# jjfiv/fastrank

Measured on AMD Instinct MI355X. Metric: coordinate-ascent NDCG@10 evals/sec on MSLR-WEB30K shape, higher is better.
Workload: dtype f64; 1 GPU; synthetic MSLR-WEB30K shape: 3800000 docs x 136 features x 31000 queries, coordinate ascent NDCG@10, 32 restarts/GPU x 25 steps/coord (configs[2]); restarts_total=32, parallelism=restart-sharded x1 (dataset replicated), launcher=single process

## Files before the change

fastrank_amd/clib.py:

```python
import ctypes as C
import json
import os
from typing import Dict, List, Optional, Set

from . import _build

_MODEL_TYPES = ["SingleFeature", "Linear", "DecisionTree", "Ensemble"]


ALLREDUCE_SUM_FN = C.CFUNCTYPE(C.c_int, C.c_void_p, C.POINTER(C.c_double), C.c_size_t)


class _CResult(C.Structure):
    _fields_ = [("error_message", C.c_void_p), ("success", C.c_void_p)]


_lib = None


def _load():
    global _lib
    if _lib is not None:
        return _lib
    path = _build.LIB_PATH
# ... 52 lines not shown
        "fr_debug_lambda_gradients_opts": (vp, [vp, vp, vp, C.c_char_p, C.c_double, vp, sz, C.c_char_p, vp, vp, sz]),
        "fr_evaluate_dense": (vp, [vp, vp, vp, C.c_char_p, vp, sz, C.POINTER(vp)]),
        "fr_rank_order": (vp, [vp, vp, vp, sz, vp, sz]),
        "fr_dataset_num_queries": (sz, [vp]),
        "fr_dataset_num_instances": (sz, [vp]),
        "fr_dataset_device_info": (vp, [vp]),
        "fr_evaluate_candidates": (vp, [vp, vp, C.c_char_p, sz, vp, vp, vp, vp, vp, vp]),
        "fr_profile_enable": (None, [C.c_int]),
        "fr_profile_reset": (None, []),
        "fr_profile_json": (vp, []),
        "fr_debug_resident_bound": (C.c_double, [C.c_int, C.c_double, C.c_double, C.c_double]),
        "fr_synchronize": (C.c_int, []),
        "fr_debug_device_plan": (vp, [C.c_char_p, C.c_int, C.c_uint32, C.c_int]),
        "fr_debug_fullrank_class": (C.c_uint32, [C.c_uint32]),
        "fr_debug_restart_queue": (vp, [C.c_uint32, C.c_uint32, C.c_uint32, vp, C.c_uint32]),
        "fr_dataset_release_replicas": (sz, [vp]),
        "fr_debug_peer_copy": (vp, [C.c_int, C.c_int, sz]),
        "fr_pack_restart_records": (vp, [C.c_char_p, sz, sz, vp]),
        "fr_unpack_restart_records": (vp, [vp, sz, sz]),
        "fr_rccl_allgather": (vp, [vp, sz, vp, sz, vp]),
        "fr_debug_rccl_selftest": (vp, [C.c_int]),
        "fr_debug_walk_tiles": (vp, [vp, vp, vp, sz, vp, vp, sz, sz]),
        "fr_debug_device_form": (vp, [vp, C.c_int, C.c_char_p, vp, sz]),
    }
    for name, (restype, argtypes) in sigs.items():
        fn = getattr(L, name)
        fn.restype = restype
        fn.argtypes = argtypes
    _lib = L
    return L
# ... 283 lines not shown
```

fastrank_amd/csrc/capi.cpp:

```cpp
#include <atomic>
#include <limits>
#include <chrono>
#include <cstdio>
#include <cstdlib>
#include <cstring>
#include <fstream>

#include "../../include/fastrank.h"
#include "host.hpp"
#include "loader.hpp"
#include "lambdamart.hpp"
#include "rf_train.hpp"

using fr::FrError;
using frjson::Value;

struct CDataset {
    std::shared_ptr<fr::DatasetView> view;
};
struct CModel {
    fr::Model actual;
};
struct CQRel {
    fr::QRel actual;
// ... 137 lines not shown
    o.set("raw_evals", Value::uint(s.raw_evals));
    o.set("ticks", Value::uint(s.ticks));
    o.set("groups", Value::uint(s.groups));
    o.set("seconds", Value::number(s.seconds));
    o.set("path", Value::string(s.path));
    o.set("restarts", Value::uint(s.restarts));
    o.set("verify_pairs", Value::uint(s.verify_pairs));
    o.set("verify_redone", Value::uint(s.verify_redone));
    o.set("exact_ticks", Value::uint(s.exact_ticks));
    o.set("exact_groups", Value::uint(s.exact_groups));
    o.set("verify_redo_entries", Value::uint(s.verify_redo_entries));
    o.set("chain_runs", Value::uint(s.chain_runs));
    o.set("chain_visits", Value::uint(s.chain_visits));
    o.set("rank_slots_on", Value::uint(s.rank_slots_on));
    o.set("rank_slots_off", Value::uint(s.rank_slots_off));
    o.set("line_searches", Value::uint(s.line_searches));
    o.set("audit_values", Value::uint(s.audit_values));
    o.set("audit_mismatches", Value::uint(s.audit_mismatches));
    o.set("devices", Value::uint(s.devices));
    o.set("refills", Value::uint(s.refills));
    if (s.device >= 0) o.set("device", Value::uint((uint64_t)s.device));
    return o;
}

enum class Learner { CoordinateAscent, RandomForest, LambdaMART };

struct ParsedRequest {
    std::string measure;
    Learner learner = Learner::CoordinateAscent;
    fr::CAParams ca;
// ... 300 lines not shown
    const std::vector<double>& exchanged = rccl.ran ? via_rccl : blocks;
    std::vector<fr::RestartResult> hist = fr::unpack_restart_records(exchanged.data(), k * cap, dim, R);
    fr::TrainStats total = stats[0];
    total.rccl_set = true;
    total.rccl = rccl;
    for (size_t i = 0; i < k; i++) {
        if (i == 0) continue;
        total.useful_evals += stats[i].useful_evals, total.raw_evals += stats[i].raw_evals;
        total.ticks = std::max(total.ticks, stats[i].ticks), total.groups += stats[i].groups;
        total.restarts += stats[i].restarts, total.refills += stats[i].refills;
        total.verify_pairs += stats[i].verify_pairs, total.verify_redone += stats[i].verify_redone;
        total.line_searches += stats[i].line_searches, total.exact_ticks += stats[i].exact_ticks;
        total.exact_groups += stats[i].exact_groups, total.verify_redo_entries += stats[i].verify_redo_entries;
        total.chain_runs += stats[i].chain_runs, total.chain_visits += stats[i].chain_visits;
        total.rank_slots_on += stats[i].rank_slots_on, total.rank_slots_off += stats[i].rank_slots_off;
        total.audit_values += stats[i].audit_values, total.audit_mismatches += stats[i].audit_mismatches;
    }
    total.seconds = std::chrono::duration<double>(std::chrono::steady_clock::now() - t0).count();
    total.devices = (uint32_t)k;
    total.device = -1;
    set_last_stats(total, stats);
    return fr::ca_select(hist, rq.ca.output_ensemble);
}

fr::Model train_rf(const std::shared_ptr<fr::DatasetView>& view, const ParsedRequest& rq) {
    auto t0 = std::chrono::steady_clock::now();
    fr::Evaluator ev = fr::make_evaluator(*view, rq.measure, rq.has_qrel ? &rq.qrel : nullptr);
    fr::RFTrainer trainer(view, std::move(ev), rq.rf);
    std::vector<fr::RFTrainer::DevicePart> parts;
    if (rq.rf.num_trees > 0) {
// ... 419 lines not shown
                ticks[w]++;
                for (auto& p : live[w]) p.left--;
                live[w].erase(std::remove_if(live[w].begin(), live[w].end(), [](const Place& p) { return p.left == 0; }), live[w].end());
                fill(w);
            }
        }
        Value o = Value::object(), ord = Value::array(), tk = Value::array();
        for (uint32_t w = 0; w < n_workers; w++) {
            Value a = Value::array();
            for (uint32_t id : order[w]) a.push(Value::uint(id));
            ord.push(std::move(a));
            tk.push(Value::uint(ticks[w]));
        }
        o.set("order", std::move(ord));
        o.set("ticks", std::move(tk));
        return frjson::dump(o);
    });
}

size_t fr_dataset_release_replicas(const CDataset* dataset) {
    if (!dataset || !dataset->view) return 0;
    std::lock_guard<std::mutex> lk(api_mu_of(*dataset));
    size_t n = 0;
    for (fr::DatasetView* v = dataset->view.get(); v; v = v->parent.get()) n += v->release_replicas();
    return n;
}

const void* fr_debug_device_plan(const void* devices_csv, int device_count, uint32_t num_restarts, int primary_device) {
    return json_call([&]() {
        const std::string csv = accept_str("devices_csv", devices_csv);
// ... 684 lines not shown
```

fastrank_amd/csrc/device.hpp:

```cpp
#pragma once
#include <algorithm>
#include <cstddef>
#include <cstdint>
#include <memory>
#include <string>
#include <utility>
#include <vector>

namespace frdev {

const char* path_env(const char* name);
inline const char* pricing_env(const char* name) {
#ifdef FR_PRICING
    return path_env(name);
#else
    (void)name;
    return nullptr;
#endif
}

enum Measure : int { M_NDCG = 0, M_AP = 1, M_RR = 2 };

constexpr uint32_t WALK_TILE = 128;
struct WalkTileLayout {
// ... 45 lines not shown
            const size_t t0 = wts[u], t1 = std::min<size_t>((size_t)wts[u + 1], t0 + WT);
            const size_t lo = std::max(b, t0) - t0, hi = std::min(e, t1) - t0;
            for (size_t p = t0 + lo; p < t0 + hi; p++) {
                out.seg[p] = (uint16_t)(lo | (hi << 8));
                out.wofs[p] = (uint8_t)(p - t0);
            }
        }
    }
    return out;
}

inline double resident_err_refresh(uint32_t d, double T) { return 1.1 * (double)(d + 1) * 0x1p-53 * T; }
inline double resident_err_update(double err, double norm, double T) { return 1.002 * err / norm + 8.0 * 0x1p-53 * T * (1.0 + 1e-6); }
inline double resident_eps_extra(double err, double norm, double T) { return 1.01 * err / norm + 10.0 * 0x1p-53 * T; }

enum : int {
    FLAG_NAN_SCORE = 1,
    FLAG_ACTUAL_GT_IDEAL = 2,
};

struct HostCSR {
    size_t n = 0, d = 0, nq = 0;
    const float* x = nullptr;
    std::vector<uint32_t> perm;
    std::vector<uint32_t> qoff;
    std::vector<float> gain;
};

struct FlatTrees {
    std::vector<int32_t> fid, lhs, rhs;
// ... 62 lines not shown
    struct LsCounts {
        unsigned long long pairs = 0, redone = 0;
    };
    bool linesearch_submit(int ctx, int measure, int64_t depth, const double* norms, const std::vector<LineGroup>& groups,
                           std::string* err);
    bool linesearch_collect(int ctx, std::vector<double>* means, LsCounts* counts, std::string* err);
    bool linesearch(int measure, int64_t depth, const double* norms, const std::vector<LineGroup>& groups,
                    std::vector<double>* means, LsCounts* counts, std::string* err);
    uint64_t resident_reserve(size_t slots, std::string* err);
    bool resident_store_from_scores(uint64_t owner, size_t slot, size_t b, std::string* err);
    const std::vector<double>& column_absmax() const;
    unsigned long long exact_fallbacks() const;
    void routing_counters(unsigned long long* exact_groups, unsigned long long* redo_entries) const;
    void chain_counters(unsigned long long* runs, unsigned long long* visits, unsigned long long* ranked_on = nullptr,
                        unsigned long long* ranked_off = nullptr) const;
    void audit_counters(unsigned long long* values, unsigned long long* mismatches) const;
    bool download_last_matrix(std::vector<double>* out, size_t* ldm, std::string* err);

    struct RfActive { uint32_t tree, key, n; };
    struct RfCand { double position, importance; uint32_t ids_i, flags, pos_l, pos_r; double sum_l, sum_r; };
    struct RfSplit { int32_t fslot; uint32_t pos, left, right; };
    bool rf_set_presence(const uint32_t* bits_by_instance, size_t words, size_t n_instances, std::string* err);
    bool rf_begin(const std::vector<uint32_t>& root_off, const std::vector<uint32_t>& root_ids, uint32_t nf,
                  const std::vector<uint32_t>& feats, std::string* err, const uint32_t* positions = nullptr,
                  bool lambda_targets = false);
    bool rf_positions(const std::vector<uint32_t>& root_ids, uint32_t* positions , std::string* err);
    bool rf_root_outputs(std::vector<double>* out, std::string* err);
    bool rf_level(const std::vector<RfActive>& active, const std::vector<uint32_t>& slot_of_key, uint32_t k, int method,
                  uint32_t min_leaf, std::vector<RfCand>* cands, std::vector<float>* label_minmax, std::string* err);
    bool rf_split(const std::vector<RfSplit>& splits, std::vector<double>* child_out, std::string* err);
// ... 81 lines not shown
```

fastrank_amd/csrc/device_dataset.inc:

```

static constexpr int LS_CONTEXTS = DeviceDataset::LINESEARCH_CONTEXTS;

static double fv_class_cost(int ci) {
    static const int sort_ce[] = {63, 191, 384, 543, 849, 1056}, merge_ce[] = {32, 80, 144, 192, 304, 336};
    const uint32_t nl = FV_CLASSES[ci].nl, pl = FV_CLASSES[ci].pl;
    const int ni = (int)nl / 16 - 1;
    uint32_t rounds = 0;
    while ((1u << rounds) < pl) rounds++;
    double c = 2.0 * nl + 2.0 * sort_ce[ni] + 5.0 * nl + (double)nl * pl;
    for (uint32_t r = 1; r <= rounds; r++) c += 5.0 * r * nl + 2.0 * merge_ce[ni];
    static const double lane_penalty[] = {1.0, 1.1, 1.25, 1.6, 2.0, 2.4};
    return c * pl * lane_penalty[rounds];
}

static int fv_class_of(uint32_t len) {
    static const bool pow2_only = [] {
        const char* e = frdev::pricing_env("FR_FV_CLASSES");
        return e != nullptr && std::strcmp(e, "pow2") == 0;
    }();
    int best = -1;
    double best_cost = 0.0;
    for (int ci = 0; ci < FV_NCLASSES; ci++) {
        const uint32_t nl = FV_CLASSES[ci].nl, pl = FV_CLASSES[ci].pl, npad = nl * pl;
        if (npad < len) continue;
// ... 52 lines not shown
        LsKind kind = LSK_TOPK;
        TickStage ts;
        LSArgs a;
        RRArgs ra;
        FSArgs fsa;
        RMArgs rma;
        DevBuf<double> fv_rows;
        size_t ldm = 0, maxc = 0, lds = 0;
        int64_t depth = 0;
        int measure = 0;
        int xs_used = 1;
        bool xs_pinned = false;
        bool audit = false;
        std::vector<LineGroup> agroups;
        unsigned redo_grid = 512, redo_grid_used = 512;
        size_t nverify = 0;
        std::vector<uint32_t> gorder, gredo_h;
        std::vector<int> gslot;
        std::vector<LineGroup> pgroups;
        std::vector<double> exact_means;
        LsCounts counts;
    };
    LsCtx ls[LS_CONTEXTS + 1];
    hipEvent_t res_ready = nullptr;
    bool res_ready_set = false;
    const double* last_M = nullptr;
    DevBuf<uint32_t> sub_idx;
    DevBuf<double> sub_partial, sub_means;
    uint32_t sub_na = 0, sub_nb = 0;
    bool ls_submit(LsCtx& c, int path, int measure, int64_t depth, const double* norms, const std::vector<LineGroup>& groups,
// ... 53 lines not shown
    DevBuf<uint8_t> wofs;
    DevBuf<uint32_t> wlist;
    std::vector<uint32_t> wt_start_h;
    size_t nwt = 0, nwlist = 0;
    std::vector<double> colstd;
    std::vector<uint8_t> colmode;
    std::vector<ColStats> colstats_h;
    DevBuf<uint8_t> rslot;
    std::vector<uint16_t> slot_rank_age;
    std::vector<uint16_t> slot_rank_upd;
    std::vector<uint16_t> slot_rank_gap;
    std::vector<uint8_t> slot_rank_mode;
    std::vector<uint16_t> slot_rate_n;
    std::vector<float> slot_rate;
    unsigned long long rank_slots_on = 0, rank_slots_off = 0;
    bool build_order_tables(std::string* err);
    DevBuf<float> xcol;
    bool build_columns(std::string* err);
    DevBuf<uint16_t> gkey;
    uint32_t key_bits = 0, key_cls_bits = 0;
    uint64_t dup_groups = 0;
    DevBuf<float> xb, gain;
    DevBuf<double> gexp, disc;
    DevBuf<uint32_t> qstart, qlen, qtight, perm, rank, run_q0, run_q1, run_pos, run_docs, run_order, gcls, qlist;
    struct SizeClass {
        uint32_t npad, offset, count;
    };
    std::vector<SizeClass> size_classes;
    std::vector<SizeClass> fv_classes;
    DevBuf<uint32_t> fv_qlist;
// ... 914 lines not shown
    copy(m.run_q0, sm.run_q0, "replicate run_q0");
    copy(m.run_q1, sm.run_q1, "replicate run_q1");
    copy(m.run_pos, sm.run_pos, "replicate run_pos");
    copy(m.run_docs, sm.run_docs, "replicate run_docs");
    copy(m.run_order, sm.run_order, "replicate run_order");
    copy(m.run_lo, sm.run_lo, "replicate run_lo");
    copy(m.gcls, sm.gcls, "replicate gcls");
    copy(m.gkey, sm.gkey, "replicate gkey");
    copy(m.segtab, sm.segtab, "replicate segtab");
    copy(m.wt_start, sm.wt_start, "replicate wt_start");
    copy(m.run_wt0, sm.run_wt0, "replicate run_wt0");
    copy(m.wofs, sm.wofs, "replicate wofs");
    m.wt_start_h = sm.wt_start_h;
    m.nwt = sm.nwt;
    m.verify_xs = sm.verify_xs;
    auto copy_optional = [&](auto& dst, const auto& from, const char* what, const char* degraded) {
        if (!ok || from.p == nullptr || from.cap == 0) return;
        std::string e2;
        if (!dst.ensure(from.cap, &e2)) {
            (void)hipGetLastError();
            warn_degraded(degraded);
            return;
        }
        ok = chk(hipMemcpyPeerAsync(dst.p, device, from.p, sm.device, from.bytes(), m.stream), what);
    };
    copy_optional(m.xcol, sm.xcol, "replicate xcol", "a device replica has no HBM for the column-major copy of the matrix: its line searches form their sums from the tiles");
    copy_optional(m.xslot, sm.xslot, "replicate xslot", "a device replica has no HBM for the visiting-order tables: its NDCG@k verify kernel walks in storage order");
    m.colstd = sm.colstd;
    m.colmode = sm.colmode;
    m.colstats_h = sm.colstats_h;
// ... 136 lines not shown
    m.xslot.alias(pm.xslot);
    m.segtab.alias(pm.segtab);
    m.wt_start.alias(pm.wt_start);
    m.wofs.alias(pm.wofs);
    m.wt_start_h = pm.wt_start_h;
    m.nwt = pm.nwt;
    m.nwlist = wlist.size();
    m.xcol.alias(pm.xcol);
    m.colstd = pm.colstd;
    m.colmode = pm.colmode;
    m.colstats_h = pm.colstats_h;
    m.dup_groups = pm.dup_groups;
    m.key_bits = pm.key_bits;
    m.key_cls_bits = pm.key_cls_bits;
    m.verify_xs = pm.verify_xs;
    m.perm.alias(pm.perm);
    m.disc.alias(pm.disc);
    m.dcgtab.alias(pm.dcgtab);
    m.termtab.alias(pm.termtab);
    if (!upload(m.qstart, qstart, err) || !upload(m.qlen, qlen, err) || !upload(m.qtight, qtight, err) ||
        !upload(m.run_q0, run_q0, err) || !upload(m.run_q1, run_q1, err) || !upload(m.run_pos, run_pos, err) ||
        !upload(m.run_docs, run_docs, err) || !upload(m.run_order, run_order, err) || !upload(m.run_lo, run_lo, err) ||
        !upload(m.qlist, qlist, err) || !upload(m.fv_qlist, fv_qlist, err) || !upload(m.qnpos, qnpos, err) ||
        !upload(m.qnneg, qnneg, err) || !upload(m.vtiles, vtiles, err) || !upload(m.run_wt0, run_wt0, err) || !upload(m.wlist, wlist, err))
        return nullptr;
    m.nvtiles = frdev::pricing_env("FR_VIEW_ALL_TILES") ? 0 : vtiles.size();
    if (!m.flags.ensure(1, err) || !m.dbgc.ensure(4, err)) return nullptr;
    if (!chk(hipMemset(m.flags.p, 0, sizeof(int)), "clear flags")) return nullptr;
    m.qstart_h = qstart;
    m.qlen_h = qlen;
    m.qnpos_h = qnpos;
    m.qnneg_h = qnneg;
    return ds;
}

static bool launch_means(const double* M, size_t ldm, size_t ncols, size_t nq, bool sums_only, DevBuf<double>& partial,
                         DevBuf<double>& means, hipStream_t st, std::string* err, const void* tail_count = nullptr,
                         const int* tail_flags = nullptr, double* host_copy = nullptr, const uint32_t* tail_groups = nullptr) {
    if (tail_count != nullptr && host_copy == nullptr) return false;
    const size_t nseg = (nq + MEAN_SEG - 1) / MEAN_SEG;
    if (!partial.ensure(std::max<size_t>(1, nseg) * ldm, err) || !means.ensure(ldm + mean_tail_words(ldm), err)) return false;
    {
        ProfScope ps("segment_sum_kernel", st);
        dim3 grid((unsigned)nseg, (unsigned)((ncols + 63) / 64));
        segment_sum_kernel<<<grid, 64, 0, st>>>(M, (uint32_t)ldm, (uint32_t)ncols, (uint32_t)nq, partial.p);
    }
    {
        ProfScope ps("final_mean_kernel", st);
        final_mean_kernel<<<dim3((unsigned)((ncols + 63) / 64)), 64, 0, st>>>(partial.p, (uint32_t)ldm, (uint32_t)ncols,
                                                                              (uint32_t)nseg, (uint32_t)(sums_only ? (nq ? 1 : 0) : nq), means.p,
                                                                              static_cast<const unsigned long long*>(tail_count), tail_flags, host_copy,
                                                                              tail_groups);
    }
    FR_HIP(hipGetLastError());
    return true;
}

static inline dim3 grid1d(size_t n, unsigned bs) { return dim3((unsigned)((n + bs - 1) / bs)); }

bool DeviceDataset::score_linear(size_t B, const double* weights, std::string* err) {
    Impl& m = *impl_;
    std::lock_guard<std::mutex> lk(m.mu);
    if (!m.bind(err)) return false;
    if (B == 0) return true;
    const size_t dp = m.dq * 4;
    if (!m.scores.ensure(B * m.np, err) || !m.weights.ensure(B * dp, err)) return false;
    m.scores_slots = B;
// ... 794 lines not shown
    return true;
}

bool DeviceDataset::Impl::tick_upload(LsCtx& c, bool with_eps2, std::string* err) {
    Impl& m = *this;
    if (with_eps2) std::memcpy(c.th<double>(c.ts.o_eps2), m.eps2_host.data(), c.ts.G * 64 * sizeof(double));
    if (m.res_ready_set && c.stream != m.stream) FR_HIP(hipStreamWaitEvent(c.stream, m.res_ready, 0));
    FR_HIP(hipMemcpyAsync(c.tick_d.p, c.tick_h.p, c.ts.total, hipMemcpyHostToDevice, c.stream));
    return true;
}
bool DeviceDataset::Impl::ls_means(LsCtx& c, std::string* err) {
    Impl& m = *this;
    const size_t ldm = c.ldm;
    if (!c.tick_res.ensure((ldm + mean_tail_words(ldm)) * sizeof(double), err)) return false;
    return launch_means(c.M.p, ldm, ldm, m.nq, m.sums_only, c.partial, c.means, c.stream, err, c.td<unsigned long long>(c.ts.o_count),
                        c.flags.p, reinterpret_cast<double*>(c.tick_res.p), c.kind == LSK_TOPK ? c.td<uint32_t>(c.ts.o_gredo) : nullptr);
}

bool DeviceDataset::Impl::tick_finish(LsCtx& c, size_t ldm, std::vector<double>* means, uint32_t* nredo, std::string* err,
                                      uint32_t* npairs, std::vector<uint32_t>* by_group) {
    Impl& m = *this;
    const size_t tail = ldm * sizeof(double);
    hipStream_t st = c.stream;
    FR_HIP(hipStreamSynchronize(st));
    means->resize(ldm);
    std::memcpy(means->data(), c.tick_res.p, tail);
    unsigned long long words[2] = {0, 0};
    std::memcpy(words, c.tick_res.p + tail, sizeof(words));
    *nredo = (uint32_t)words[0];
    if (npairs) *npairs = (uint32_t)(words[0] >> 32);
    if (by_group) {
// ... 148 lines not shown
        else if (xs == 2) linesearch_verify_kernel<K, 1, true, 2><<<grid, dim3(WAVE), tab_lds, st>>>(a);
        else if (xs == 3 || K < 10) linesearch_verify_kernel<K, 1, true, 3><<<grid, dim3(WAVE), tab_lds, st>>>(a);
        else linesearch_verify_kernel<K, 1, true, (K < 10 ? 3 : 4)><<<grid, dim3(WAVE), tab_lds, st>>>(a);
    } else {
        const dim3 grid((unsigned)(nruns8 * ((G + 1) / 2)));
        linesearch_verify_kernel<K, 2, false><<<grid, dim3(WAVE), 2 * dp * sizeof(double) + tab_lds, st>>>(a);
    }
}

uint64_t DeviceDataset::resident_reserve(size_t slots, std::string* err) {
    Impl& m = *impl_;
    std::lock_guard<std::mutex> lk(m.mu);
    if (!m.bind(err)) return 0;
    m.res_owner++;
    m.verify_xs = std::max(1, m.verify_xs - 1);
    m.res_half.clear();
    if (m.xcol.p == nullptr) {
        if (err) *err = "resident_reserve: the dataset has no column-major copy";
        return 0;
    }
    m.slot_exact_left.assign(slots, 0);
    m.slot_backoff.assign(slots, 0);
    {
        std::string* e2 = err;
        auto ensure = [&]() -> bool { return m.res.ensure(slots * 2 * m.np, e2); };
        if (!ensure()) return 0;
    }
    m.res_half.assign(slots, 0);
    m.slot_rank_age.assign(slots, 0xFFFF);
    m.slot_rank_upd.assign(slots, 0);
    m.slot_rank_gap.assign(slots, 1);
    m.slot_rank_mode.assign(slots, 1);
    m.slot_rate_n.assign(slots, 0);
    m.slot_rate.assign(slots, 0.0f);
    if (m.xslot.p != nullptr) {
        std::string e2;
        if (m.rslot.ensure(slots * m.np, &e2)) {
            rslot_identity_kernel<<<dim3(1024), dim3(256), 0, m.stream>>>(m.rslot.p, m.wofs.p, m.np, slots * m.np);
            if (hipGetLastError() != hipSuccess) m.rslot.release();
        } else {
            (void)hipGetLastError();
        }
    }
    return m.res_owner;
}

bool DeviceDataset::resident_store_from_scores(uint64_t owner, size_t slot, size_t b, std::string* err) {
// ... 25 lines not shown
    *mismatches = impl_->audit_mismatches;
}

unsigned long long DeviceDataset::exact_fallbacks() const {
    std::lock_guard<std::mutex> lk(impl_->mu);
    return impl_->exact_fallbacks;
}

void DeviceDataset::chain_counters(unsigned long long* runs, unsigned long long* visits, unsigned long long* ranked_on,
                                   unsigned long long* ranked_off) const {
    std::lock_guard<std::mutex> lk(impl_->mu);
    *runs = impl_->chain_runs;
    *visits = impl_->chain_visits;
    if (ranked_on) *ranked_on = impl_->rank_slots_on;
    if (ranked_off) *ranked_off = impl_->rank_slots_off;
}

void DeviceDataset::routing_counters(unsigned long long* exact_groups, unsigned long long* redo_entries) const {
    std::lock_guard<std::mutex> lk(impl_->mu);
    *exact_groups = impl_->exact_groups;
    *redo_entries = impl_->approx_redo_entries;
}

static void launch_scores(const FSArgs& a, size_t maxc, unsigned nblocks, size_t lds, hipStream_t st) {
    if (maxc <= 16) linesearch_scores_kernel<16, 16><<<dim3(nblocks), dim3(WAVE), lds, st>>>(a);
    else if (maxc <= 51) linesearch_scores_kernel<51, 16><<<dim3(nblocks), dim3(WAVE), lds, st>>>(a);
    else linesearch_scores_kernel<64, 16><<<dim3(nblocks), dim3(WAVE), lds, st>>>(a);
}

FSArgs DeviceDataset::Impl::scores_args(const uint32_t* gf, const double* w, const double* cand, double* rows, int* fl, size_t gc) const {
// ... 743 lines not shown
    FR_HIP(hipGetLastError());
    unsigned long long bad = 0;
    FR_HIP(hipMemcpyAsync(&bad, m.audit_cnt.p, sizeof(bad), hipMemcpyDeviceToHost, m.stream));
    FR_HIP(hipStreamSynchronize(m.stream));
    m.audit_values += ncells;
    m.audit_mismatches += bad;
    return true;
}

bool DeviceDataset::Impl::topk_policy(LsCtx& c, uint32_t nredo, uint32_t nslices, std::string* err) {
    Impl& m = *this;
    const size_t ldm = c.ldm, G = ldm / 64, nV = c.nverify;
    const std::vector<uint32_t>& by_group = c.gredo_h;
    LSArgs& a = c.a;
    const unsigned grid_used = c.redo_grid_used;
    if (nredo > grid_used / 2) c.redo_grid = std::min(8192u, std::max(c.redo_grid, 512u) * 4u);
    else if (nredo < grid_used / 16 && c.redo_grid > 512u) c.redo_grid /= 2u;
    m.approx_redo_entries += nslices;
    for (size_t k = 0; k < nV; k++) m.chain_runs += by_group[G + k];
    m.chain_visits += (unsigned long long)m.n * nV;
    {
        static const double t_off = [] {
            const char* e = frdev::pricing_env("FR_RANK_OFF_BELOW");
            return e ? std::atof(e) : RANK_OFF_BELOW;
        }();
        static const double t_on = [] {
            const char* e = frdev::pricing_env("FR_RANK_ON_ABOVE");
            return e ? std::atof(e) : RANK_ON_ABOVE;
        }();
        std::vector<double> runs(m.slot_rank_mode.size(), 0.0), visits(m.slot_rank_mode.size(), 0.0);
        for (size_t k = 0; k < nV; k++) {
            const int slot = c.gslot[k];
// ... 4 lines not shown
        for (size_t slot = 0; slot < runs.size(); slot++) {
            if (visits[slot] == 0.0) continue;
            const double r = runs[slot] / visits[slot];
            uint16_t& n = m.slot_rate_n[slot];
            if (n < 16) n++;
            m.slot_rate[slot] += (float)((r - (double)m.slot_rate[slot]) / (double)n);
            if (n < 16) continue;
            if (m.slot_rank_mode[slot] == 1 && (double)m.slot_rate[slot] < t_off) {
                m.slot_rank_mode[slot] = 2;
                m.rank_slots_off++;
            } else if (m.slot_rank_mode[slot] == 2 && (double)m.slot_rate[slot] > t_on) {
                m.slot_rank_mode[slot] = 1;
                m.rank_slots_on++;
            }
        }
    }
    if (c.audit) {
        const size_t nel = m.nq * ldm;
        if (!m.audit.ensure(nel, err) || !m.audit_cnt.ensure(1, err)) return false;
        FR_HIP(hipMemcpyAsync(m.audit.p, c.M.p, nel * sizeof(double), hipMemcpyDeviceToDevice, c.stream));
        LSArgs x = a;
        x.work_list = nullptr;
        x.work_count = nullptr;
        x.g_base = 0;
        x.G = (uint32_t)G;
        dispatch_exact(x, c.depth, (unsigned)(((m.nruns + 7) / 8) * 8 * G), c.maxc, c.lds, c.stream);
        FR_HIP(hipMemsetAsync(m.audit_cnt.p, 0, sizeof(unsigned long long), c.stream));
        audit_compare_kernel<<<dim3(1024), dim3(256), 0, c.stream>>>(m.audit.p, c.M.p, nel, m.audit_cnt.p);
        unsigned long long bad = 0;
        FR_HIP(hipMemcpyAsync(&bad, m.audit_cnt.p, sizeof(bad), hipMemcpyDeviceToHost, c.stream));
// ... 1128 lines not shown
```

fastrank_amd/csrc/host.hpp:

```cpp
#pragma once
#include <algorithm>
#include <atomic>
#include <charconv>
#include <chrono>
#include <cmath>
#include <cstdint>
#include <cstdio>
#include <cstdlib>
#include <functional>
#include <map>
#include <memory>
#include <mutex>
#include <set>
#include <string>
#include <thread>
#include <unordered_map>
#include <vector>

#include "device.hpp"
#include "json.hpp"

namespace fr {

using frjson::Value;
// ... 742 lines not shown
    uint64_t useful_evals = 0;
    uint64_t raw_evals = 0;
    uint64_t ticks = 0;
    uint64_t groups = 0;
    double seconds = 0.0;
    std::string path;
    uint32_t restarts = 0;
    uint64_t verify_pairs = 0, verify_redone = 0;
    uint64_t line_searches = 0;
    uint64_t audit_values = 0, audit_mismatches = 0;
    uint64_t exact_ticks = 0;
    uint64_t exact_groups = 0;
    uint64_t verify_redo_entries = 0;
    uint64_t chain_runs = 0, chain_visits = 0;
    uint64_t rank_slots_on = 0, rank_slots_off = 0;
    uint32_t devices = 1;
    uint32_t refills = 0;
    int device = -1;
    bool rccl_set = false;
    frdev::RcclReport rccl;
};

struct ExactTickCount {
    frdev::DeviceDataset& dev;
    TrainStats& st;
    unsigned long long base, av0 = 0, am0 = 0, eg0 = 0, re0 = 0, cr0 = 0, cv0 = 0, on0 = 0, off0 = 0;
    ExactTickCount(frdev::DeviceDataset& d, TrainStats& s) : dev(d), st(s), base(d.exact_fallbacks()) {
        d.audit_counters(&av0, &am0);
        d.routing_counters(&eg0, &re0);
        d.chain_counters(&cr0, &cv0, &on0, &off0);
// ... 129 lines not shown
            path_ = caps[0] == caps[2] ? LS_TOPK : (caps[1] == caps[2] ? LS_FULLRANK : LS_NONE);
        }
        stats_.path = path_ == LS_TOPK ? "fused_linesearch" : (path_ == LS_FULLRANK ? "fused_fullrank" : "generic_sort");
        stats_.restarts = (uint32_t)rs_.size();
        if (rs_.empty()) return;
        const size_t R = rs_.size();
        std::vector<size_t> all(R);
        for (size_t k = 0; k < R; k++) all[k] = k;
        init_restarts(all);
        const char* res_env = frdev::path_env("FR_LS_RESIDENT");
        if (path_ != LS_NONE && !(res_env && res_env[0] == '0')) {
            std::string _err;
            res_owner_ = dev.resident_reserve(R, &_err);
            if (res_owner_ != 0) {
                resident_ = true;
                if (const char* e = frdev::path_env("FR_RESIDENT_REFRESH")) res_refresh_ = (uint32_t)std::max(1, atoi(e));
                for (size_t k = 0; k < R; k++) rs_[k].slot = (int)k;
                refresh_resident(all);
            }
        }
    }

    bool done() const {
        for (const Restart& r : rs_)
            if (!r.done) return false;
        return !queue_ || queue_->empty();
    }

    bool tick() {
        refill();
// ... 423 lines not shown
```

fastrank_amd/csrc/kernels_metric.inc:

```
__device__ __forceinline__ bool key_before(double sa, uint32_t ia, double sb, uint32_t ib) {
    if (ia == IDX_INVALID) return false;
    if (ib == IDX_INVALID) return true;
    if (sa > sb) return true;
    if (sa < sb) return false;
    return ia > ib;
}

__global__ __launch_bounds__(256) void metric_sort_kernel(
    const double* __restrict__ scores, uint32_t np, const uint32_t* __restrict__ qstart,
    const uint32_t* __restrict__ qlen, const uint32_t* __restrict__ qtight, const double* __restrict__ gexp,
    const float* __restrict__ gain, const double* __restrict__ disc, const double* __restrict__ norms, int measure,
    int depth, uint32_t B, double* __restrict__ M, uint32_t* __restrict__ rank_out, const uint32_t* __restrict__ perm,
    int* __restrict__ flags, uint32_t npad_max, const uint32_t* __restrict__ qlist, uint32_t b_off,
    double* gkeys, uint32_t* gidx) {
    extern __shared__ double lds_raw[];
    double* keys = lds_raw;
    uint32_t* idx = (uint32_t*)(keys + npad_max);
    if (gkeys != nullptr) {
        const size_t slab = ((size_t)blockIdx.y * gridDim.x + blockIdx.x) * npad_max;
        keys = gkeys + slab;
        idx = gidx + slab;
    }
    const uint32_t q = qlist[blockIdx.x], b = blockIdx.y + b_off, tid = threadIdx.x, nt = blockDim.x;
    const uint32_t base = qstart[q], n = qlen[q];
// ... 84 lines not shown
                        sum_precision += keys[i];
                        in_list++;
                    }
                }
                if (num_rel == 0) num_rel = in_list;
                if (num_rel != 0) result = sum_precision / (double)num_rel;
            }
        }
    }
    if (tid == 0) M[(size_t)q * B + b] = result;
}

constexpr uint32_t MEAN_SEG = 256;

__global__ __launch_bounds__(64) void segment_sum_kernel(const double* __restrict__ M, uint32_t ldm, uint32_t ncols,
                                                         uint32_t nq, double* __restrict__ partial) {
    const uint32_t c = blockIdx.y * blockDim.x + threadIdx.x;
    const uint32_t s = blockIdx.x;
    if (c >= ncols) return;
    const uint32_t q0 = s * MEAN_SEG;
    const uint32_t q1 = (q0 + MEAN_SEG < nq) ? q0 + MEAN_SEG : nq;
    const double* p = M + (size_t)q0 * ldm + c;
    double sum = 0.0;
    uint32_t q = q0;
    for (; q + 16 <= q1; q += 16) {
        double v[16];
#pragma unroll
        for (int t = 0; t < 16; t++) v[t] = p[(size_t)t * ldm];
#pragma unroll
        for (int t = 0; t < 16; t++) sum += v[t];
        p += (size_t)16 * ldm;
    }
    for (; q < q1; q++) {
        sum += *p;
        p += ldm;
    }
    partial[(size_t)s * ldm + c] = sum;
}

__host__ __device__ constexpr size_t mean_tail_words(size_t ldm) { return 2 + ldm / 64; }
__global__ void final_mean_kernel(const double* __restrict__ partial, uint32_t ldm, uint32_t ncols, uint32_t nseg,
                                  uint32_t div, double* __restrict__ means, const unsigned long long* __restrict__ tail_count,
                                  const int* __restrict__ tail_flags, double* __restrict__ host_copy,
                                  const uint32_t* __restrict__ tail_groups) {
    uint32_t c = blockIdx.x * blockDim.x + threadIdx.x;
    if (c == 0 && tail_count != nullptr) {
        const unsigned long long w0 = *tail_count, w1 = (unsigned long long)(unsigned int)*tail_flags;
        reinterpret_cast<unsigned long long*>(means)[ldm] = w0;
        reinterpret_cast<unsigned long long*>(means)[ldm + 1] = w1;
        if (host_copy != nullptr) {
            reinterpret_cast<unsigned long long*>(host_copy)[ldm] = w0;
            reinterpret_cast<unsigned long long*>(host_copy)[ldm + 1] = w1;
        }
    }
    if (tail_groups != nullptr && c < 2 * (ldm / 64)) {
        const uint32_t v = tail_groups[c];
        reinterpret_cast<uint32_t*>(means + ldm + 2)[c] = v;
        if (host_copy != nullptr) reinterpret_cast<uint32_t*>(host_copy + ldm + 2)[c] = v;
    }
    if (c >= ncols) return;
    double sum = 0.0;
    uint32_t s = 0;
    const double* p = partial + c;
    for (; s + 16 <= nseg; s += 16) {
        double v[16];
#pragma unroll
        for (int t = 0; t < 16; t++) v[t] = p[(size_t)(s + t) * ldm];
#pragma unroll
        for (int t = 0; t < 16; t++) sum += v[t];
    }
    for (; s < nseg; s++) sum += p[(size_t)s * ldm];
    const double mean = div ? sum / (double)div : 0.0;
    means[c] = mean;
    if (host_copy != nullptr) host_copy[c] = mean;
}

__global__ __launch_bounds__(MEAN_SEG) void subset_segment_sum_kernel(const double* __restrict__ M, uint32_t ldm,
                                                                      const uint32_t* __restrict__ idx, uint32_t n_a, uint32_t n_b,
// ... 34 lines not shown
```

fastrank_amd/native.py:

```python
import ctypes as C
import json
from typing import Dict, List, Optional, Tuple

import numpy as np

from .clib import ALLREDUCE_SUM_FN, CDataset, CModel, CQRel, _json_reply, _load, _status, _take_str, _unwrap


def device_count() -> int:
    return int(_load().fr_device_count())


def set_device(ordinal: int) -> None:
    if _load().fr_set_device(int(ordinal)) != 0:
        raise RuntimeError("fr_set_device({}) failed".format(ordinal))


def version() -> str:
    return _load().fr_version().decode("utf-8")


def synchronize() -> None:
    if _load().fr_synchronize() != 0:
        raise RuntimeError("device synchronize failed")
# ... 305 lines not shown
    return model


def select_model(restarts: List[Dict], output_ensemble: bool = False) -> CModel:
    payload = json.dumps(restarts).encode("utf-8")
    return CModel(_unwrap(_load().fr_select_model(payload, 1 if output_ensemble else 0)))


def device_plan(devices: str, device_count: int, num_restarts: int, primary_device: int = 0) -> Dict:
    return _json_reply(_load().fr_debug_device_plan(devices.encode("utf-8"), device_count, num_restarts, primary_device))


def restart_queue_replay(num_restarts: int, n_workers: int, capacity: int, lengths) -> Dict:
    arr = np.ascontiguousarray(lengths, dtype=np.uint32)
    return _json_reply(_load().fr_debug_restart_queue(int(num_restarts), int(n_workers), int(capacity), arr.ctypes.data, len(arr)))


def peer_copy(src_device: int, dst_device: int, nbytes: int = 256 << 20) -> Dict:
    return _json_reply(_load().fr_debug_peer_copy(int(src_device), int(dst_device), int(nbytes)))


def pack_restart_records(restarts: List[Dict], cap: int, dim: int) -> "np.ndarray":
    out = np.zeros((int(cap), 3 + int(dim)), dtype=np.float64)
    _status(_load().fr_pack_restart_records(json.dumps(restarts).encode("utf-8"), int(cap), int(dim), out.ctypes.data))
    return out


def unpack_restart_records(records: "np.ndarray", dim: int) -> List[Dict]:
    arr = np.ascontiguousarray(records, dtype=np.float64).reshape(-1, 3 + int(dim))
    return _json_reply(_load().fr_unpack_restart_records(arr.ctypes.data, arr.shape[0], int(dim)))
# ... 162 lines not shown
```

include/fastrank.h:

```cpp
#ifndef FASTRANK_AMD_H
#define FASTRANK_AMD_H

#include <stddef.h>
#include <stdint.h>

#ifdef __cplusplus
extern "C" {
#endif

typedef struct CDataset CDataset;
typedef struct CModel CModel;
typedef struct CQRel CQRel;

typedef struct CResult {
    const void *error_message;
    const void *success;
} CResult;


void free_str(void *originally_from_library);
void free_c_result(CResult *originally_from_library);
void free_dataset(CDataset *originally_from_library);
void free_model(CModel *originally_from_library);
void free_cqrel(CQRel *originally_from_library);
// ... 82 lines not shown
size_t fr_dataset_num_queries(const CDataset *dataset);
size_t fr_dataset_num_instances(const CDataset *dataset);

const void *fr_evaluate_candidates(const CDataset *dataset, const CQRel *qrel, const void *evaluator_name,
                                   size_t n_groups, const uint32_t *features, const double *base_weights,
                                   const uint32_t *n_cand, const double *candidates, double *out_means,
                                   double *out_per_query);

void fr_profile_enable(int on);
void fr_profile_reset(void);
const void *fr_profile_json(void);
int fr_synchronize(void);
double fr_debug_resident_bound(int which, double a, double b, double c);
uint32_t fr_debug_fullrank_class(uint32_t len);
const void *fr_debug_device_plan(const void *devices_csv, int device_count, uint32_t num_restarts, int primary_device);
const void *fr_debug_restart_queue(uint32_t num_restarts, uint32_t n_workers, uint32_t capacity, const uint32_t *lengths,
                                   uint32_t n_lengths);
const void *fr_debug_peer_copy(int src_device, int dst_device, size_t bytes);
const void *fr_pack_restart_records(const void *restarts_json, size_t cap, size_t dim, double *out);
const void *fr_unpack_restart_records(const double *records, size_t n_records, size_t dim);
const void *fr_rccl_allgather(const int *devices, size_t n, const double *blocks, size_t block_len, double *out);
const void *fr_debug_walk_tiles(const uint32_t *run_pos, const uint32_t *run_q0, const uint32_t *run_q1, size_t nruns,
                                const uint32_t *qstart, const uint32_t *qlen, size_t nq, size_t np);
const void *fr_debug_device_form(const CDataset *dataset, int slot, const void *table, void *out, size_t out_bytes);
const void *fr_debug_rccl_selftest(int device);
size_t fr_dataset_release_replicas(const CDataset *dataset);

#ifdef __cplusplus
}
#endif
// ... 2 lines not shown
```

Before: 709,100 evals/s.

## Skip unused candidate columns in means, remember rank mode, smooth redo grid

The segment-sum and final-mean kernels now skip columns beyond each group's candidate count for top-k line searches, so padded columns are no longer summed. Rank-slot mode is remembered across resident reservations: if most slots ended in the off mode, new slots start off. The redo grid size is now taken from a 16-tick history maximum with a lower floor of 32 instead of the old grow/shrink rule with a floor of 512. These changes add state carried across calls and a debug replay entry point, and risk undersized redo grids or early-return divergence inside the kernels.

```diff
diff --git a/fastrank_amd/clib.py b/fastrank_amd/clib.py
--- a/fastrank_amd/clib.py
+++ b/fastrank_amd/clib.py
@@ -90,6 +90,7 @@
         "fr_debug_device_plan": (vp, [C.c_char_p, C.c_int, C.c_uint32, C.c_int]),
         "fr_debug_fullrank_class": (C.c_uint32, [C.c_uint32]),
         "fr_debug_restart_queue": (vp, [C.c_uint32, C.c_uint32, C.c_uint32, vp, C.c_uint32]),
+        "fr_debug_tick_tail": (vp, [vp, vp, vp, sz, C.c_int, vp, sz]),
         "fr_dataset_release_replicas": (sz, [vp]),
         "fr_debug_peer_copy": (vp, [C.c_int, C.c_int, sz]),
         "fr_pack_restart_records": (vp, [C.c_char_p, sz, sz, vp]),
diff --git a/fastrank_amd/csrc/capi.cpp b/fastrank_amd/csrc/capi.cpp
--- a/fastrank_amd/csrc/capi.cpp
+++ b/fastrank_amd/csrc/capi.cpp
@@ -175,6 +175,7 @@
     o.set("chain_visits", Value::uint(s.chain_visits));
     o.set("rank_slots_on", Value::uint(s.rank_slots_on));
     o.set("rank_slots_off", Value::uint(s.rank_slots_off));
+    o.set("rank_slots_start_off", Value::uint(s.rank_slots_start_off));
     o.set("line_searches", Value::uint(s.line_searches));
     o.set("audit_values", Value::uint(s.audit_values));
     o.set("audit_mismatches", Value::uint(s.audit_mismatches));
@@ -505,6 +506,7 @@
         total.exact_groups += stats[i].exact_groups, total.verify_redo_entries += stats[i].verify_redo_entries;
         total.chain_runs += stats[i].chain_runs, total.chain_visits += stats[i].chain_visits;
         total.rank_slots_on += stats[i].rank_slots_on, total.rank_slots_off += stats[i].rank_slots_off;
+        total.rank_slots_start_off += stats[i].rank_slots_start_off;
         total.audit_values += stats[i].audit_values, total.audit_mismatches += stats[i].audit_mismatches;
     }
     total.seconds = std::chrono::duration<double>(std::chrono::steady_clock::now() - t0).count();
@@ -954,6 +956,30 @@
         }
         o.set("order", std::move(ord));
         o.set("ticks", std::move(tk));
+        return frjson::dump(o);
+    });
+}
+
+const void* fr_debug_tick_tail(const uint8_t* modes, const float* rates, const uint16_t* rate_n, size_t slots, int prev_off,
+                               const uint32_t* redo_counts, size_t n_counts) {
+    return json_call([&]() {
+        if ((slots > 0 && (!modes || !rates || !rate_n)) || (n_counts > 0 && !redo_counts)) fr::fail_str("fr_debug_tick_tail: bad arguments");
+        frdev::RankMemory prev;
+        prev.off = prev_off != 0;
+        const frdev::RankMemory mem = frdev::rank_memory_verdict(modes, rates, rate_n, slots, prev);
+        const frdev::RankMemory view = mem;
+        Value o = Value::object(), grids = Value::array();
+        o.set("memory_off", Value::boolean(mem.off));
+        o.set("memory_rate", Value::number((double)mem.rate));
+        o.set("start_mode", Value::uint(mem.start_mode()));
+        o.set("view_start_mode", Value::uint(view.start_mode()));
+        uint32_t hist[frdev::REDO_HISTORY] = {};
+        for (size_t t = 0; t < n_counts; t++) {
+            grids.push(Value::uint(frdev::redo_grid_rule(hist, frdev::REDO_HISTORY)));
+            hist[t % frdev::REDO_HISTORY] = redo_counts[t];
+        }
+        grids.push(Value::uint(frdev::redo_grid_rule(hist, frdev::REDO_HISTORY)));
+        o.set("grids", std::move(grids));
         return frjson::dump(o);
     });
 }
diff --git a/fastrank_amd/csrc/device.hpp b/fastrank_amd/csrc/device.hpp
--- a/fastrank_amd/csrc/device.hpp
+++ b/fastrank_amd/csrc/device.hpp
@@ -83,6 +83,37 @@
 inline double resident_err_update(double err, double norm, double T) { return 1.002 * err / norm + 8.0 * 0x1p-53 * T * (1.0 + 1e-6); }
 inline double resident_eps_extra(double err, double norm, double T) { return 1.01 * err / norm + 10.0 * 0x1p-53 * T; }
 
+struct RankMemory {
+    bool off = false;
+    float rate = 0.0f;
+    uint8_t start_mode() const { return off ? 2 : 1; }
+};
+inline RankMemory rank_memory_verdict(const uint8_t* modes, const float* rates, const uint16_t* rate_n, size_t slots, RankMemory prev) {
+    if (slots == 0) return prev;
+    size_t off = 0, measured = 0;
+    double sum = 0.0;
+    for (size_t s = 0; s < slots; s++) {
+        off += modes[s] == 2;
+        if (rate_n[s] > 0) {
+            sum += (double)rates[s];
+            measured++;
+        }
+    }
+    RankMemory r;
+    r.off = off * 4 >= slots * 3;
+    r.rate = measured ? (float)(sum / (double)measured) : prev.rate;
+    return r;
+}
+
+constexpr unsigned REDO_HISTORY = 16, REDO_GRID_MIN = 32, REDO_GRID_MAX = 8192;
+inline unsigned redo_grid_rule(const uint32_t* hist, size_t n) {
+    uint64_t mx = 0;
+    for (size_t i = 0; i < n; i++) mx = hist[i] > mx ? hist[i] : mx;
+    unsigned g = REDO_GRID_MIN;
+    while (g < REDO_GRID_MAX && (uint64_t)g < mx * 4) g *= 2;
+    return g;
+}
+
 enum : int {
     FLAG_NAN_SCORE = 1,
     FLAG_ACTUAL_GT_IDEAL = 2,
@@ -175,6 +206,7 @@
     void routing_counters(unsigned long long* exact_groups, unsigned long long* redo_entries) const;
     void chain_counters(unsigned long long* runs, unsigned long long* visits, unsigned long long* ranked_on = nullptr,
                         unsigned long long* ranked_off = nullptr) const;
+    size_t rank_start_off(bool* memory_off = nullptr, float* memory_rate = nullptr) const;
     void audit_counters(unsigned long long* values, unsigned long long* mismatches) const;
     bool download_last_matrix(std::vector<double>* out, size_t* ldm, std::string* err);
 
diff --git a/fastrank_amd/csrc/device_dataset.inc b/fastrank_amd/csrc/device_dataset.inc
--- a/fastrank_amd/csrc/device_dataset.inc
+++ b/fastrank_amd/csrc/device_dataset.inc
@@ -90,6 +90,8 @@
         bool audit = false;
         std::vector<LineGroup> agroups;
         unsigned redo_grid = 512, redo_grid_used = 512;
+        uint32_t redo_hist[REDO_HISTORY] = {};
+        unsigned redo_hist_at = 0;
         size_t nverify = 0;
         std::vector<uint32_t> gorder, gredo_h;
         std::vector<int> gslot;
@@ -173,6 +175,8 @@
     std::vector<uint16_t> slot_rate_n;
     std::vector<float> slot_rate;
     unsigned long long rank_slots_on = 0, rank_slots_off = 0;
+    RankMemory rank_mem;
+    size_t rank_start_off = 0;
     bool build_order_tables(std::string* err);
     DevBuf<float> xcol;
     bool build_columns(std::string* err);
@@ -1117,6 +1121,7 @@
     m.wt_start_h = sm.wt_start_h;
     m.nwt = sm.nwt;
     m.verify_xs = sm.verify_xs;
+    m.rank_mem = sm.rank_mem;
     auto copy_optional = [&](auto& dst, const auto& from, const char* what, const char* degraded) {
         if (!ok || from.p == nullptr || from.cap == 0) return;
         std::string e2;
@@ -1283,6 +1288,7 @@
     m.key_bits = pm.key_bits;
     m.key_cls_bits = pm.key_cls_bits;
     m.verify_xs = pm.verify_xs;
+    m.rank_mem = pm.rank_mem;
     m.perm.alias(pm.perm);
     m.disc.alias(pm.disc);
     m.dcgtab.alias(pm.dcgtab);
@@ -1305,21 +1311,22 @@
 
 static bool launch_means(const double* M, size_t ldm, size_t ncols, size_t nq, bool sums_only, DevBuf<double>& partial,
                          DevBuf<double>& means, hipStream_t st, std::string* err, const void* tail_count = nullptr,
-                         const int* tail_flags = nullptr, double* host_copy = nullptr, const uint32_t* tail_groups = nullptr) {
+                         const int* tail_flags = nullptr, double* host_copy = nullptr, const uint32_t* tail_groups = nullptr,
+                         const uint32_t* gncand = nullptr) {
     if (tail_count != nullptr && host_copy == nullptr) return false;
     const size_t nseg = (nq + MEAN_SEG - 1) / MEAN_SEG;
     if (!partial.ensure(std::max<size_t>(1, nseg) * ldm, err) || !means.ensure(ldm + mean_tail_words(ldm), err)) return false;
     {
         ProfScope ps("segment_sum_kernel", st);
         dim3 grid((unsigned)nseg, (unsigned)((ncols + 63) / 64));
-        segment_sum_kernel<<<grid, 64, 0, st>>>(M, (uint32_t)ldm, (uint32_t)ncols, (uint32_t)nq, partial.p);
+        segment_sum_kernel<<<grid, 64, 0, st>>>(M, (uint32_t)ldm, (uint32_t)ncols, (uint32_t)nq, partial.p, gncand);
     }
     {
         ProfScope ps("final_mean_kernel", st);
         final_mean_kernel<<<dim3((unsigned)((ncols + 63) / 64)), 64, 0, st>>>(partial.p, (uint32_t)ldm, (uint32_t)ncols,
                                                                               (uint32_t)nseg, (uint32_t)(sums_only ? (nq ? 1 : 0) : nq), means.p,
                                                                               static_cast<const unsigned long long*>(tail_count), tail_flags, host_copy,
-                                                                              tail_groups);
+                                                                              tail_groups, gncand);
     }
     FR_HIP(hipGetLastError());
     return true;
@@ -2144,7 +2151,8 @@
     const size_t ldm = c.ldm;
     if (!c.tick_res.ensure((ldm + mean_tail_words(ldm)) * sizeof(double), err)) return false;
     return launch_means(c.M.p, ldm, ldm, m.nq, m.sums_only, c.partial, c.means, c.stream, err, c.td<unsigned long long>(c.ts.o_count),
-                        c.flags.p, reinterpret_cast<double*>(c.tick_res.p), c.kind == LSK_TOPK ? c.td<uint32_t>(c.ts.o_gredo) : nullptr);
+                        c.flags.p, reinterpret_cast<double*>(c.tick_res.p), c.kind == LSK_TOPK ? c.td<uint32_t>(c.ts.o_gredo) : nullptr,
+                        c.kind == LSK_TOPK && !frdev::pricing_env("FR_MEAN_ALL_COLUMNS") ? c.td<uint32_t>(c.ts.o_gncand) : nullptr);
 }
 
 bool DeviceDataset::Impl::tick_finish(LsCtx& c, size_t ldm, std::vector<double>* means, uint32_t* nredo, std::string* err,
@@ -2323,6 +2331,9 @@
     if (!m.bind(err)) return 0;
     m.res_owner++;
     m.verify_xs = std::max(1, m.verify_xs - 1);
+    const bool rank_env = frdev::pricing_env("FR_RANK_OFF_BELOW") != nullptr || frdev::pricing_env("FR_RANK_ON_ABOVE") != nullptr ||
+                          frdev::pricing_env("FR_RANK_MEMORY_OFF") != nullptr;
+    const uint8_t start_mode = rank_env ? (uint8_t)1 : m.rank_mem.start_mode();
     m.res_half.clear();
     if (m.xcol.p == nullptr) {
         if (err) *err = "resident_reserve: the dataset has no column-major copy";
@@ -2339,7 +2350,8 @@
     m.slot_rank_age.assign(slots, 0xFFFF);
     m.slot_rank_upd.assign(slots, 0);
     m.slot_rank_gap.assign(slots, 1);
-    m.slot_rank_mode.assign(slots, 1);
+    m.slot_rank_mode.assign(slots, start_mode);
+    m.rank_start_off = start_mode == 2 ? slots : 0;
     m.slot_rate_n.assign(slots, 0);
     m.slot_rate.assign(slots, 0.0f);
     if (m.xslot.p != nullptr) {
@@ -2395,6 +2407,13 @@
     *visits = impl_->chain_visits;
     if (ranked_on) *ranked_on = impl_->rank_slots_on;
     if (ranked_off) *ranked_off = impl_->rank_slots_off;
+}
+
+size_t DeviceDataset::rank_start_off(bool* memory_off, float* memory_rate) const {
+    std::lock_guard<std::mutex> lk(impl_->mu);
+    if (memory_off) *memory_off = impl_->rank_mem.off;
+    if (memory_rate) *memory_rate = impl_->rank_mem.rate;
+    return impl_->rank_start_off;
 }
 
 void DeviceDataset::routing_counters(unsigned long long* exact_groups, unsigned long long* redo_entries) const {
@@ -3168,8 +3187,13 @@
     const std::vector<uint32_t>& by_group = c.gredo_h;
     LSArgs& a = c.a;
     const unsigned grid_used = c.redo_grid_used;
-    if (nredo > grid_used / 2) c.redo_grid = std::min(8192u, std::max(c.redo_grid, 512u) * 4u);
-    else if (nredo < grid_used / 16 && c.redo_grid > 512u) c.redo_grid /= 2u;
+    (void)grid_used;
+    c.redo_hist[c.redo_hist_at++ % REDO_HISTORY] = nredo;
+    static const unsigned grid_floor = [] {
+        const char* e = frdev::pricing_env("FR_REDO_FLOOR");
+        return e ? (unsigned)std::max(1, std::atoi(e)) : REDO_GRID_MIN;
+    }();
+    c.redo_grid = std::max(grid_floor, redo_grid_rule(c.redo_hist, REDO_HISTORY));
     m.approx_redo_entries += nslices;
     for (size_t k = 0; k < nV; k++) m.chain_runs += by_group[G + k];
     m.chain_visits += (unsigned long long)m.n * nV;
@@ -3204,6 +3228,7 @@
                 m.rank_slots_on++;
             }
         }
+        m.rank_mem = rank_memory_verdict(m.slot_rank_mode.data(), m.slot_rate.data(), m.slot_rate_n.data(), m.slot_rank_mode.size(), m.rank_mem);
     }
     if (c.audit) {
         const size_t nel = m.nq * ldm;
diff --git a/fastrank_amd/csrc/host.hpp b/fastrank_amd/csrc/host.hpp
--- a/fastrank_amd/csrc/host.hpp
+++ b/fastrank_amd/csrc/host.hpp
@@ -780,6 +780,7 @@
     uint64_t verify_redo_entries = 0;
     uint64_t chain_runs = 0, chain_visits = 0;
     uint64_t rank_slots_on = 0, rank_slots_off = 0;
+    uint64_t rank_slots_start_off = 0;
     uint32_t devices = 1;
     uint32_t refills = 0;
     int device = -1;
@@ -939,6 +940,7 @@
             res_owner_ = dev.resident_reserve(R, &_err);
             if (res_owner_ != 0) {
                 resident_ = true;
+                stats_.rank_slots_start_off = dev.rank_start_off();
                 if (const char* e = frdev::path_env("FR_RESIDENT_REFRESH")) res_refresh_ = (uint32_t)std::max(1, atoi(e));
                 for (size_t k = 0; k < R; k++) rs_[k].slot = (int)k;
                 refresh_resident(all);
diff --git a/fastrank_amd/csrc/kernels_metric.inc b/fastrank_amd/csrc/kernels_metric.inc
--- a/fastrank_amd/csrc/kernels_metric.inc
+++ b/fastrank_amd/csrc/kernels_metric.inc
@@ -122,10 +122,12 @@
 constexpr uint32_t MEAN_SEG = 256;
 
 __global__ __launch_bounds__(64) void segment_sum_kernel(const double* __restrict__ M, uint32_t ldm, uint32_t ncols,
-                                                         uint32_t nq, double* __restrict__ partial) {
+                                                         uint32_t nq, double* __restrict__ partial,
+                                                         const uint32_t* __restrict__ gncand) {
     const uint32_t c = blockIdx.y * blockDim.x + threadIdx.x;
     const uint32_t s = blockIdx.x;
     if (c >= ncols) return;
+    if (gncand != nullptr && threadIdx.x >= gncand[blockIdx.y]) return;
     const uint32_t q0 = s * MEAN_SEG;
     const uint32_t q1 = (q0 + MEAN_SEG < nq) ? q0 + MEAN_SEG : nq;
     const double* p = M + (size_t)q0 * ldm + c;
@@ -150,7 +152,7 @@
 __global__ void final_mean_kernel(const double* __restrict__ partial, uint32_t ldm, uint32_t ncols, uint32_t nseg,
                                   uint32_t div, double* __restrict__ means, const unsigned long long* __restrict__ tail_count,
                                   const int* __restrict__ tail_flags, double* __restrict__ host_copy,
-                                  const uint32_t* __restrict__ tail_groups) {
+                                  const uint32_t* __restrict__ tail_groups, const uint32_t* __restrict__ gncand) {
     uint32_t c = blockIdx.x * blockDim.x + threadIdx.x;
     if (c == 0 && tail_count != nullptr) {
         const unsigned long long w0 = *tail_count, w1 = (unsigned long long)(unsigned int)*tail_flags;
@@ -170,6 +172,7 @@
     double sum = 0.0;
     uint32_t s = 0;
     const double* p = partial + c;
+    if (gncand != nullptr && (c & 63u) >= gncand[c >> 6]) s = nseg;
     for (; s + 16 <= nseg; s += 16) {
         double v[16];
 #pragma unroll
diff --git a/fastrank_amd/native.py b/fastrank_amd/native.py
--- a/fastrank_amd/native.py
+++ b/fastrank_amd/native.py
@@ -343,6 +343,16 @@
 def restart_queue_replay(num_restarts: int, n_workers: int, capacity: int, lengths) -> Dict:
     arr = np.ascontiguousarray(lengths, dtype=np.uint32)
     return _json_reply(_load().fr_debug_restart_queue(int(num_restarts), int(n_workers), int(capacity), arr.ctypes.data, len(arr)))
+
+
+def tick_tail_replay(modes, rates, rate_n, prev_off: bool, redo_counts) -> Dict:
+    m = np.ascontiguousarray(modes, dtype=np.uint8)
+    r = np.ascontiguousarray(rates, dtype=np.float32)
+    k = np.ascontiguousarray(rate_n, dtype=np.uint16)
+    c = np.ascontiguousarray(redo_counts, dtype=np.uint32)
+    assert len(m) == len(r) == len(k)
+    return _json_reply(_load().fr_debug_tick_tail(m.ctypes.data if len(m) else None, r.ctypes.data if len(m) else None, k.ctypes.data if len(m) else None,
+                                                  len(m), 1 if prev_off else 0, c.ctypes.data if len(c) else None, len(c)))
 
 
 def peer_copy(src_device: int, dst_device: int, nbytes: int = 256 << 20) -> Dict:
diff --git a/include/fastrank.h b/include/fastrank.h
--- a/include/fastrank.h
+++ b/include/fastrank.h
@@ -120,6 +120,8 @@
 double fr_debug_resident_bound(int which, double a, double b, double c);
 uint32_t fr_debug_fullrank_class(uint32_t len);
 const void *fr_debug_device_plan(const void *devices_csv, int device_count, uint32_t num_restarts, int primary_device);
+const void *fr_debug_tick_tail(const uint8_t *modes, const float *rates, const uint16_t *rate_n, size_t slots, int prev_off,
+                               const uint32_t *redo_counts, size_t n_counts);
 const void *fr_debug_restart_queue(uint32_t num_restarts, uint32_t n_workers, uint32_t capacity, const uint32_t *lengths,
                                    uint32_t n_lengths);
 const void *fr_debug_peer_copy(int src_device, int dst_device, size_t bytes);
```

New measurement: 710,600 evals/s, median of 2. About the same (+0.2%).
